# Kizuna42/office-person-detection-vit

Measured on AMD Instinct MI355X. Metric: frames/sec (Phase-2 DETR detect) at 800x1333 batch 8, higher is better.
Workload: dtype f16

## Files before the change

office_person_detection_vit_amd/csrc/kernels_btail3.hip:

```cpp
#include <hip/hip_runtime.h>
#include "opd_kernels.h"
#include "opd_elem.h"

typedef elem_t half8 __attribute__((ext_vector_type(8)));
typedef float float4v __attribute__((ext_vector_type(4)));
typedef unsigned int uint2v __attribute__((ext_vector_type(2)));
typedef unsigned int uint4v __attribute__((ext_vector_type(4)));

namespace {

constexpr int ROW_BYTES = 128;

__device__ __forceinline__ int swz(int row, int chunk) { return row * ROW_BYTES + ((chunk ^ (row & 7)) << 4); }

__device__ __forceinline__ int xcd_logical_block(int bid, int nblocks) {
    const int q = nblocks >> 3, r = nblocks & 7;
    const int x = bid & 7, k = bid >> 3;
    return (x < r ? x * (q + 1) : r * (q + 1) + (x - r) * q) + k;
}
__device__ __forceinline__ int xcd_logical_block_rev(int bid, int nblocks) {
    const int q = nblocks >> 3, r = nblocks & 7;
    const int x = bid & 7, k = bid >> 3;
    return (x < r ? x * (q + 1) + q - k : r * (q + 1) + (x - r) * q + q - 1 - k);
}
__device__ __forceinline__ int fdiv(const int m, const FastDiv& f) { return f.one ? m : (int)(__umulhi((unsigned)m, f.mul) >> f.shift); }

__device__ __forceinline__ unsigned pack2h(float a, float b) {
    typedef elem_t half2v __attribute__((ext_vector_type(2)));
    half2v h;
    h[0] = (elem_t)a;
    h[1] = (elem_t)b;
    unsigned u;
    __builtin_memcpy(&u, &h, 4);
    return u;
}
__device__ __forceinline__ void unpack2h(unsigned u, float& a, float& b) {
    typedef elem_t half2v __attribute__((ext_vector_type(2)));
    half2v h;
    __builtin_memcpy(&h, &u, 4);
    a = (float)h[0];
    b = (float)h[1];
}
__device__ __forceinline__ half8 as_half8(unsigned a, unsigned b, unsigned c, unsigned d) {
    uint4v u = {a, b, c, d};
    half8 h;
    __builtin_memcpy(&h, &u, 16);
    return h;
}
template <int N_OUTSTANDING>
__device__ __forceinline__ void wait_vmcnt() {
    static_assert(N_OUTSTANDING >= 0 && N_OUTSTANDING <= 63, "vmcnt range");
    asm volatile("s_waitcnt vmcnt(%0)" ::"n"(N_OUTSTANDING) : "memory");
}
__device__ __forceinline__ void compiler_fence() { asm volatile("" ::: "memory"); }
__device__ __forceinline__ void lds_barrier() { asm volatile("s_waitcnt lgkmcnt(0)\n\ts_barrier" ::: "memory"); }

constexpr int W2BUF = 0, W3BUF = 65536, XBUF = 131072, EXBUF = 98304;
constexpr int STAGE_BYTES = 49152;
constexpr int LDS_BYTES = 163840;

template <int C3, bool TRACE = false>
__global__ __launch_bounds__(512) void btail256_kernel(BtailParams p) {
#if defined(__HIP_DEVICE_COMPILE__)
    unsigned long long tstamp[16] = {};
    auto stamp = [&](const int i) {
        if constexpr (TRACE) asm volatile("s_memtime %0\n\ts_waitcnt lgkmcnt(0)" : "=s"(tstamp[i])::"memory");
    };
    if constexpr (TRACE) asm volatile("s_memrealtime %0\n\ts_waitcnt lgkmcnt(0)" : "=s"(tstamp[0])::"memory");
    stamp(1);
    extern __shared__ __attribute__((aligned(16))) unsigned char smem[];
    constexpr int C1 = 256, C2 = 1024, NCH = C2 / 64;
    static_assert(C3 == 0 || C3 == 256, "reduce width");
    const int tid = threadIdx.x;
    const int lane = tid & 63;
    const int wave = __builtin_amdgcn_readfirstlane(tid >> 6);
    const int pair = wave >> 1, half = wave & 1;
    const int g = lane >> 4, li = lane & 15;
    const int m_base = (p.rev ? xcd_logical_block_rev(blockIdx.x, gridDim.x) : xcd_logical_block(blockIdx.x, gridDim.x)) * 128;

    const int lrow = lane >> 3;
    const int lchunk = (lane & 7) ^ lrow;
    const unsigned backoff = (unsigned)(p.W + 1) * (unsigned)C1 * 2u;
    const __amdgpu_buffer_rsrc_t rsrc_a = __builtin_amdgcn_make_buffer_rsrc(
        const_cast<char*>(reinterpret_cast<const char*>(p.x1)) - backoff, 0, (unsigned)((size_t)p.B * p.H * p.W * C1 * 2) + backoff, 0x00020000);
    const __amdgpu_buffer_rsrc_t rsrc_w1 = __builtin_amdgcn_make_buffer_rsrc(const_cast<f16_t*>(p.w1), 0, (unsigned)(C1 * 9 * C1 * 2), 0x00020000);
    const __amdgpu_buffer_rsrc_t rsrc_w2 = __builtin_amdgcn_make_buffer_rsrc(const_cast<f16_t*>(p.w2p), 0, (unsigned)(C2 * C1 * 2), 0x00020000);
    const __amdgpu_buffer_rsrc_t rsrc_w3 = __builtin_amdgcn_make_buffer_rsrc(const_cast<f16_t*>(C3 ? p.w3p : p.w2p), 0, (unsigned)((C3 ? C3 : 1) * C2 * 2), 0x00020000);
    unsigned rowoff[2], rowmask[2], woff1[4], woff2[4], woff3[4];
    {
        const int ohw = p.OH * p.OW;
#pragma unroll
        for (int i = 0; i < 2; ++i) {
            const int m = m_base + (wave * 2 + i) * 8 + lrow;
            const bool okm = m < p.M;
            const int mm = okm ? m : 0;
            const int b = fdiv(mm, p.fd_ohw);
            const int r = mm - b * ohw;
            const int oh = fdiv(r, p.fd_ow);
            const int ow = r - oh * p.OW;
            rowoff[i] = (unsigned)(((b * p.H + oh * p.stride) * p.W + ow * p.stride) * C1) * 2u + (unsigned)lchunk * 16u;
            unsigned kwmask = 0, mask = 0;
#pragma unroll
            for (int kw = 0; kw < 3; ++kw)
                if ((unsigned)(ow * p.stride - 1 + kw) < (unsigned)p.W) kwmask |= 1u << kw;
#pragma unroll
            for (int kh = 0; kh < 3; ++kh)
                if ((unsigned)(oh * p.stride - 1 + kh) < (unsigned)p.H) mask |= kwmask << (kh * 3);
            rowmask[i] = okm ? mask : 0u;
        }
#pragma unroll
        for (int i = 0; i < 4; ++i) {
            const int q = wave * 4 + i;
            woff1[i] = (unsigned)((q * 8 + lrow) * (9 * C1)) * 2u + (unsigned)lchunk * 16u;
            woff2[i] = (unsigned)(((q & 7) * 8 + lrow) * C1 + (q >> 3) * 64) * 2u + (unsigned)lchunk * 16u;
            woff3[i] = (unsigned)((q * 8 + lrow) * C2) * 2u + (unsigned)lchunk * 16u;
        }
    }
    constexpr int kpc = C1 / 64;
    constexpr int nk = 9 * kpc;
    int tap_kh = 0, tap_kw = 0, tap_c = 0;
    int is_tap = 0, is_soff_a = 0, is_ks = 0;
    auto begin_issue = [&](int ks) {
        is_tap = tap_kh * 3 + tap_kw;
        is_soff_a = ((tap_kh * p.W + tap_kw) * C1 + tap_c * 64) * 2;
        is_ks = ks;
        if (++tap_c == kpc) {
            tap_c = 0;
            if (++tap_kw == 3) { tap_kw = 0; ++tap_kh; }
        }
    };
    auto issue_piece = [&](int i, int stage_off) {
        unsigned char* As = smem + stage_off;
        if (i < 2) {
            const unsigned vo = ((rowmask[i] >> is_tap) & 1u) ? rowoff[i] : 0x80000000u;
            __builtin_amdgcn_raw_ptr_buffer_load_lds(rsrc_a, (__attribute__((address_space(3))) void*)(As + (wave * 2 + i) * 1024), 16, vo, is_soff_a, 0, 0);
        } else {
            __builtin_amdgcn_raw_ptr_buffer_load_lds(rsrc_w1, (__attribute__((address_space(3))) void*)(As + 16384 + (wave * 4 + i - 2) * 1024), 16, woff1[i - 2], is_ks * 128, 0, 0);
        }
    };
    auto issue_main = [&](int ks, int stage_off) {
        begin_issue(ks);
#pragma unroll
        for (int i = 0; i < 6; ++i) issue_piece(i, stage_off);
    };
    auto issue_w2_piece = [&](int j, int i) {
        unsigned char* dst = smem + W2BUF + (j & 1) * 32768;
        __builtin_amdgcn_raw_ptr_buffer_load_lds(rsrc_w2, (__attribute__((address_space(3))) void*)(dst + (wave * 4 + i) * 1024), 16, woff2[i], j * (64 * C1 * 2), 0, 0);
    };
    auto issue_w3_piece = [&](int j, int i) {
        if constexpr (C3 > 0) {
            unsigned char* dst = smem + W3BUF + (j & 1) * 32768;
            __builtin_amdgcn_raw_ptr_buffer_load_lds(rsrc_w3, (__attribute__((address_space(3))) void*)(dst + (wave * 4 + i) * 1024), 16, woff3[i], j * 128, 0, 0);
        }
    };

    const int pr_m = m_base + pair * 32 + (g & 1) * 16 + li;
    const bool has_res = p.res != nullptr && !(p.dbg & 4);
    const unsigned y_bytes = (unsigned)((size_t)p.M * C2 * 2);
    const __amdgpu_buffer_rsrc_t rsrc_r = __builtin_amdgcn_make_buffer_rsrc(const_cast<f16_t*>(has_res ? p.res : p.x1), 0, has_res ? y_bytes : 0u, 0x00020000);
    const __amdgpu_buffer_rsrc_t rsrc_y = __builtin_amdgcn_make_buffer_rsrc(p.y, 0, (p.dbg & 2) ? 0u : y_bytes, 0x00020000);
    const unsigned pr_off = (unsigned)pr_m * (unsigned)(C2 * 2) + (unsigned)(half * 32 + (g >> 1) * 8) * 2u;
    auto load_res = [&](int j, uint4v (&r)[2]) {
#pragma unroll
        for (int nt = 0; nt < 2; ++nt) r[nt] = __builtin_amdgcn_raw_buffer_load_b128(rsrc_r, pr_off + (unsigned)(j * 64 + nt * 16) * 2u, 0, 0);
    };

    stamp(2);
    issue_main(0, 0);
    issue_main(1, STAGE_BYTES);
    float4v acc1[8][2];
#pragma unroll
    for (int nt = 0; nt < 8; ++nt) {
        const float4v b = *reinterpret_cast<const float4v*>(p.b1 + half * 128 + nt * 16 + g * 4);
        acc1[nt][0] = b;
        acc1[nt][1] = b;
    }
#pragma unroll
    for (int nt = 0; nt < 8; ++nt) asm volatile("" : "+v"(acc1[nt][0]), "+v"(acc1[nt][1]));
    const int group = wave >> 2;
    half8 xf[2][2], wf[2][8];
    auto read_frags = [&](int stage_off) {
        const unsigned char* As = smem + stage_off;
        const unsigned char* Ws = As + 16384;
#pragma unroll
        for (int kk = 0; kk < 2; ++kk) {
#pragma unroll
            for (int mt = 0; mt < 2; ++mt) xf[kk][mt] = *reinterpret_cast<const half8*>(As + swz(pair * 32 + mt * 16 + li, kk * 4 + g));
#pragma unroll
            for (int nt = 0; nt < 8; ++nt) wf[kk][nt] = *reinterpret_cast<const half8*>(Ws + swz(half * 128 + nt * 16 + li, kk * 4 + g));
        }
    };
    auto mfma_phase = [&](auto&& between) {
        __builtin_amdgcn_s_setprio(1);
#pragma unroll
        for (int kk = 0; kk < 2; ++kk)
#pragma unroll
            for (int nt = 0; nt < 8; ++nt) {
#pragma unroll
                for (int mt = 0; mt < 2; ++mt) acc1[nt][mt] = OPD_MFMA_16x16x32(wf[kk][nt], xf[kk][mt], acc1[nt][mt]);
                if ((nt & 3) == 3) {
                    __builtin_amdgcn_sched_barrier(0);
                    between(kk * 2 + (nt >> 2));
                    __builtin_amdgcn_sched_barrier(0);
                }
            }
        __builtin_amdgcn_s_setprio(0);
        lds_barrier();
    };
    auto no_issue = [](int) {};
    static_assert(nk % 3 == 0, "stage bookkeeping below assumes the last k-step sits in stage 2");
    wait_vmcnt<6>();
    lds_barrier();
    if (group == 1) lds_barrier();
    int st_cur = 0, st_next2 = 2 * STAGE_BYTES;
#pragma unroll 1
    for (int ks = 0; ks + 2 < nk; ++ks) {
        read_frags(st_cur);
        compiler_fence();
        begin_issue(ks + 2);
#pragma unroll
        for (int i = 0; i < 2; ++i) issue_piece(i, st_next2);
        wait_vmcnt<2>();
        lds_barrier();
        mfma_phase([&](int slot) { issue_piece(2 + slot, st_next2); });
        st_cur = st_cur == 2 * STAGE_BYTES ? 0 : st_cur + STAGE_BYTES;
        st_next2 = st_next2 == 2 * STAGE_BYTES ? 0 : st_next2 + STAGE_BYTES;
    }
    float4v acc2[2][2];
    auto load_bias2 = [&](int j) {
#pragma unroll
        for (int nt = 0; nt < 2; ++nt) acc2[nt][0] = *reinterpret_cast<const float4v*>(p.b2 + j * 64 + half * 32 + nt * 16 + g * 4);
    };
    float4v accz[C3 ? 8 : 1][2];
    read_frags(STAGE_BYTES);
    compiler_fence();
#pragma unroll
    for (int i = 0; i < 4; ++i) issue_w2_piece(0, i);
    wait_vmcnt<4>();
    lds_barrier();
    mfma_phase(no_issue);
    read_frags(2 * STAGE_BYTES);
    compiler_fence();
#pragma unroll
    for (int i = 0; i < 4; ++i) issue_w2_piece(1, i);
#pragma unroll
    for (int i = 0; i < 4; ++i) issue_w3_piece(0, i);
    compiler_fence();
    load_bias2(0);
    if constexpr (C3 > 0) {
#pragma unroll
        for (int nt = 0; nt < 8; ++nt) accz[nt][0] = *reinterpret_cast<const float4v*>(p.b3 + half * 128 + nt * 16 + g * 4);
    }
    uint4v res[3][2];
    load_res(0, res[0]);
    load_res(1, res[1]);
    compiler_fence();
    lds_barrier();
    mfma_phase(no_issue);
    if (group == 0) lds_barrier();
    wait_vmcnt<0>();
    if constexpr (C3 > 0) {
#pragma unroll
        for (int nt = 0; nt < 8; ++nt) {
            asm volatile("" : "+v"(accz[nt][0]));
            accz[nt][1] = accz[nt][0];
        }
    }
    lds_barrier();
    stamp(3);

    half8 a1[2][8];
#pragma unroll
    for (int mt = 0; mt < 2; ++mt)
#pragma unroll
        for (int kb = 0; kb < 4; ++kb) {
            float4v u = acc1[2 * kb][mt], v = acc1[2 * kb + 1][mt];
#pragma unroll
            for (int r = 0; r < 4; ++r) {
                u[r] = u[r] > 0.f ? u[r] : 0.f;
                v[r] = v[r] > 0.f ? v[r] : 0.f;
            }
            a1[mt][kb] = as_half8(pack2h(u[0], u[1]), pack2h(u[2], u[3]), pack2h(v[0], v[1]), pack2h(v[2], v[3]));
            *reinterpret_cast<half8*>(smem + EXBUF + wave * 8192 + (mt * 4 + kb) * 1024 + lane * 16) = a1[mt][kb];
        }
    lds_barrier();
#pragma unroll
    for (int mt = 0; mt < 2; ++mt)
#pragma unroll
        for (int kb = 0; kb < 4; ++kb) {
            const half8 own = a1[mt][kb];
            const half8 oth = *reinterpret_cast<const half8*>(smem + EXBUF + (wave ^ 1) * 8192 + (mt * 4 + kb) * 1024 + lane * 16);
            a1[mt][kb] = half ? oth : own;
            a1[mt][4 + kb] = half ? own : oth;
        }
    lds_barrier();
    stamp(4);
    if (p.dbg & 8) return;

#pragma unroll
    for (int j = 0; j < NCH; ++j) {
        const unsigned char* W2s = smem + W2BUF + (j & 1) * 32768;
#pragma unroll
        for (int nt = 0; nt < 2; ++nt) acc2[nt][1] = acc2[nt][0];
        {
            auto w2frag = [&](int t, int nt) {
                const int kb = t;
                return *reinterpret_cast<const half8*>(W2s + (kb >> 1) * 8192 + swz(half * 32 + nt * 16 + li, (kb & 1) * 4 + g));
            };
            half8 ring[3][2];
#pragma unroll
            for (int t = 0; t < 2; ++t)
#pragma unroll
                for (int nt = 0; nt < 2; ++nt) ring[t][nt] = w2frag(t, nt);
            __builtin_amdgcn_s_setprio(1);
#pragma unroll
            for (int t = 0; t < 8; ++t) {
                if (t + 2 < 8) {
#pragma unroll
                    for (int nt = 0; nt < 2; ++nt) ring[(t + 2) % 3][nt] = w2frag(t + 2, nt);
                }
#pragma unroll
                for (int nt = 0; nt < 2; ++nt)
#pragma unroll
                    for (int mt = 0; mt < 2; ++mt) acc2[nt][mt] = OPD_MFMA_16x16x32(ring[t % 3][nt], a1[mt][t], acc2[nt][mt]);
                __builtin_amdgcn_sched_barrier(0);
            }
            __builtin_amdgcn_s_setprio(0);
        }
        uint4v (&res_cur)[2] = res[j % 3];
        unsigned pk[2][2][2];
        uint4v yo[2];
#pragma unroll
        for (int nt = 0; nt < 2; ++nt) {
            float4v v0 = acc2[nt][0], v1 = acc2[nt][1];
            {
                uint4v r = res_cur[nt];
                asm volatile("" : "+v"(r));
                const uint2v s0 = __builtin_amdgcn_permlane16_swap(r[0], r[2], false, false);
                const uint2v s1 = __builtin_amdgcn_permlane16_swap(r[1], r[3], false, false);
                float a, b;
                unpack2h(s0[0], a, b); v0[0] += a; v0[1] += b;
                unpack2h(s1[0], a, b); v0[2] += a; v0[3] += b;
                unpack2h(s0[1], a, b); v1[0] += a; v1[1] += b;
                unpack2h(s1[1], a, b); v1[2] += a; v1[3] += b;
            }
#pragma unroll
            for (int r = 0; r < 4; ++r) {
                v0[r] = v0[r] > 0.f ? v0[r] : 0.f;
                v1[r] = v1[r] > 0.f ? v1[r] : 0.f;
            }
            pk[nt][0][0] = pack2h(v0[0], v0[1]);
            pk[nt][0][1] = pack2h(v0[2], v0[3]);
            pk[nt][1][0] = pack2h(v1[0], v1[1]);
            pk[nt][1][1] = pack2h(v1[2], v1[3]);
            const uint2v s0 = __builtin_amdgcn_permlane16_swap(pk[nt][0][0], pk[nt][1][0], false, false);
            const uint2v s1 = __builtin_amdgcn_permlane16_swap(pk[nt][0][1], pk[nt][1][1], false, false);
            yo[nt] = uint4v{s0[0], s1[0], s0[1], s1[1]};
        }
        half8 yf[2][2];
        if constexpr (C3 > 0) {
#pragma unroll
            for (int mt = 0; mt < 2; ++mt) {
                yf[0][mt] = as_half8(pk[0][mt][0], pk[0][mt][1], pk[1][mt][0], pk[1][mt][1]);
                *reinterpret_cast<half8*>(smem + XBUF + (j & 1) * 16384 + wave * 2048 + mt * 1024 + lane * 16) = yf[0][mt];
            }
        }
        wait_vmcnt<0>();
        lds_barrier();
#pragma unroll
        for (int nt = 0; nt < 2; ++nt) __builtin_amdgcn_raw_buffer_store_b128(yo[nt], rsrc_y, pr_off + (unsigned)(j * 64 + nt * 16) * 2u, 0, 0);
        if (j + 2 < NCH) load_res(j + 2, res[(j + 2) % 3]);
        if (j + 1 < NCH) load_bias2(j + 1);
        compiler_fence();
        if constexpr (C3 > 0) {
            const unsigned char* W3s = smem + W3BUF + (j & 1) * 32768;
#pragma unroll
            for (int mt = 0; mt < 2; ++mt) {
                const half8 oth = *reinterpret_cast<const half8*>(smem + XBUF + (j & 1) * 16384 + (wave ^ 1) * 2048 + mt * 1024 + lane * 16);
                const half8 own = yf[0][mt];
                yf[0][mt] = half ? oth : own;
                yf[1][mt] = half ? own : oth;
            }
            auto w3frag = [&](int idx) {
                const int kb = idx >> 3;
                return *reinterpret_cast<const half8*>(W3s + swz(half * 128 + (idx & 7) * 16 + li, kb * 4 + g));
            };
            half8 ring[4];
#pragma unroll
            for (int i = 0; i < 4; ++i) ring[i] = w3frag(i);
#pragma unroll
            for (int idx = 0; idx < 16; ++idx) {
                const half8 wf = ring[idx & 3];
#pragma unroll
                for (int mt = 0; mt < 2; ++mt) accz[idx & 7][mt] = OPD_MFMA_16x16x32(wf, yf[idx >> 3][mt], accz[idx & 7][mt]);
                if (idx + 4 < 16) ring[idx & 3] = w3frag(idx + 4);
                __builtin_amdgcn_sched_barrier(0);
                if (p.dbg & 16) {}
                else if (idx < 4) { if (j + 1 < NCH) issue_w3_piece(j + 1, idx); }
                else if (idx < 8) { if (j + 2 < NCH) issue_w2_piece(j + 2, idx - 4); }
                __builtin_amdgcn_sched_barrier(0);
            }
        } else {
            if (j + 2 < NCH) {
#pragma unroll
                for (int i = 0; i < 4; ++i) issue_w2_piece(j + 2, i);
            }
            compiler_fence();
        }
        if (j & 1) stamp(5 + (j >> 1));
    }

    if constexpr (C3 > 0) {
        const __amdgpu_buffer_rsrc_t rsrc_z = __builtin_amdgcn_make_buffer_rsrc(p.z, 0, (p.dbg & 2) ? 0u : (unsigned)((size_t)p.M * C3 * 2), 0x00020000);
        const unsigned zoff = (unsigned)pr_m * (unsigned)(C3 * 2) + (unsigned)(half * 128 + (g >> 1) * 8) * 2u;
#pragma unroll
        for (int nt = 0; nt < 8; ++nt) {
            float4v v0 = accz[nt][0], v1 = accz[nt][1];
#pragma unroll
            for (int r = 0; r < 4; ++r) {
                v0[r] = v0[r] > 0.f ? v0[r] : 0.f;
                v1[r] = v1[r] > 0.f ? v1[r] : 0.f;
            }
            const uint2v s0 = __builtin_amdgcn_permlane16_swap(pack2h(v0[0], v0[1]), pack2h(v1[0], v1[1]), false, false);
            const uint2v s1 = __builtin_amdgcn_permlane16_swap(pack2h(v0[2], v0[3]), pack2h(v1[2], v1[3]), false, false);
            const uint4v o = {s0[0], s1[0], s0[1], s1[1]};
            __builtin_amdgcn_raw_buffer_store_b128(o, rsrc_z, zoff + (unsigned)(nt * 16) * 2u, 0, 0);
        }
    }
    if constexpr (TRACE) {
        stamp(13);
        asm volatile("s_waitcnt vmcnt(0)" ::: "memory");
        stamp(14);
        asm volatile("s_memrealtime %0\n\ts_waitcnt lgkmcnt(0)" : "=s"(tstamp[15])::"memory");
        if (threadIdx.x == 0 && p.trace) {
#pragma unroll
            for (int i = 0; i < 16; ++i) p.trace[(size_t)blockIdx.x * 16 + i] = tstamp[i];
        }
    }
#endif
}

template <int C3, bool TRACE = false>
// ... 20 lines not shown
```

office_person_detection_vit_amd/csrc/kernels_btail.hip:

```cpp
#include <hip/hip_runtime.h>
#include "opd_kernels.h"
#include "opd_elem.h"

typedef elem_t half8 __attribute__((ext_vector_type(8)));
typedef float float4v __attribute__((ext_vector_type(4)));
typedef unsigned int uint2v __attribute__((ext_vector_type(2)));
typedef unsigned int uint4v __attribute__((ext_vector_type(4)));

namespace {

constexpr int ROW_BYTES = 128;
constexpr int NW = 4;

__device__ __forceinline__ int swz(int row, int chunk) { return row * ROW_BYTES + ((chunk ^ (row & 7)) << 4); }

__device__ __forceinline__ int xcd_logical_block(int bid, int nblocks) {
    const int q = nblocks >> 3, r = nblocks & 7;
    const int x = bid & 7, k = bid >> 3;
    return (x < r ? x * (q + 1) : r * (q + 1) + (x - r) * q) + k;
}

__device__ __forceinline__ int own_row(const int rho) { return (rho & ~31) | (((rho >> 2) & 3) << 3) | (((rho >> 4) & 1) << 2) | (rho & 3); }
__device__ __forceinline__ int own_ch(const int nt, const int g) { return (nt >> 1) * 32 + g * 8 + (nt & 1) * 4; }

// ... 30 lines not shown
    return h;
}

template <int N_OUTSTANDING>
__device__ __forceinline__ void wait_vmcnt() {
    static_assert(N_OUTSTANDING >= 0 && N_OUTSTANDING <= 63, "vmcnt range");
    asm volatile("s_waitcnt vmcnt(%0)" ::"n"(N_OUTSTANDING) : "memory");
}
__device__ __forceinline__ void compiler_fence() { asm volatile("" ::: "memory"); }

template <int C1, int C3, bool RDMA, bool SC = false, bool TRACE = false, int RC = 0>
__global__ __launch_bounds__(64 * NW, 8 / NW) void btail_kernel(BtailParams p) {
#if defined(__HIP_DEVICE_COMPILE__)
    unsigned long long tstamp[16] = {};
    auto stamp = [&](const int i) {
        if constexpr (TRACE) asm volatile("s_memtime %0\n\ts_waitcnt lgkmcnt(0)" : "=s"(tstamp[i])::"memory");
    };
    if constexpr (TRACE) asm volatile("s_memrealtime %0\n\ts_waitcnt lgkmcnt(0)" : "=s"(tstamp[0])::"memory");
    stamp(1);
    static_assert(!RDMA || C1 == 64, "residual staging buffers are budgeted for C1 == 64 (80 KiB of LDS per workgroup)");
    static_assert(!RDMA || RC == 0, "a rebuilt residual is not staged");
    static_assert(!SC || (C1 == 64 && !RDMA), "fused shortcut: 64-channel tails only; it replaces the residual");
    extern __shared__ __attribute__((aligned(16))) unsigned char smem[];
    constexpr int C2 = 4 * C1;
    constexpr int NT1 = C1 / 16;
    constexpr int KK1 = C1 / 32;
    constexpr int BM = 32 * NW;
    constexpr int A_BYTES = BM * ROW_BYTES;
    constexpr int RC_BYTES = RC ? 2 * 64 * ROW_BYTES : 0;
    constexpr int W1_PIECES = C1 / (8 * NW);
    constexpr int NCH = C2 / 64;
    constexpr int W2C_BYTES = 64 * C1 * 2;
    constexpr int W2_PIECES = W2C_BYTES / (1024 * NW);
    constexpr int W3_PIECES = C3 / (8 * NW);
    constexpr int SC_PIECES = 8 / NW;
    static_assert(W1_PIECES >= 1 && W2_PIECES >= 1 && (C3 == 0 || W3_PIECES >= 1), "every wave stages at least one piece of every operand");
    constexpr int NT3 = C3 / 16;
    constexpr int WSC_BYTES = SC ? 64 * ROW_BYTES : 0;
    constexpr int CHUNK_BYTES = W2C_BYTES + C3 * ROW_BYTES + WSC_BYTES + RC_BYTES;
    constexpr int STAGE_BYTES = (A_BYTES + C1 * ROW_BYTES) > CHUNK_BYTES ? (A_BYTES + C1 * ROW_BYTES) : CHUNK_BYTES;
    static_assert(RC == 0 || (RC == 1 && C1 == 64 && !RDMA && !SC), "residual rebuild: second block of stage 1");

    const int tid = threadIdx.x;
    const int lane = tid & 63;
    const int wave = __builtin_amdgcn_readfirstlane(tid >> 6);
    const int g = lane >> 4, li = lane & 15;
    const int m_base = (p.rev ? xcd_logical_block_rev(blockIdx.x, gridDim.x) : xcd_logical_block(blockIdx.x, gridDim.x)) * BM;
    const int wm0 = m_base + wave * 32;

    const int lrow = lane >> 3;
    const int lchunk = (lane & 7) ^ lrow;
    const unsigned backoff = (unsigned)(p.W + 1) * (unsigned)C1 * 2u;
    const __amdgpu_buffer_rsrc_t rsrc_a = __builtin_amdgcn_make_buffer_rsrc(
        const_cast<char*>(reinterpret_cast<const char*>(p.x1)) - backoff, 0, (unsigned)((size_t)p.B * p.H * p.W * C1 * 2) + backoff, 0x00020000);
    const __amdgpu_buffer_rsrc_t rsrc_w1 = __builtin_amdgcn_make_buffer_rsrc(const_cast<f16_t*>(p.w1), 0, (unsigned)(C1 * 9 * C1 * 2), 0x00020000);
    const __amdgpu_buffer_rsrc_t rsrc_w2 = __builtin_amdgcn_make_buffer_rsrc(const_cast<f16_t*>(p.w2p), 0, (unsigned)(C2 * C1 * 2), 0x00020000);
    const __amdgpu_buffer_rsrc_t rsrc_w3 = __builtin_amdgcn_make_buffer_rsrc(const_cast<f16_t*>(C3 ? p.w3p : p.w2p), 0, (unsigned)((C3 ? C3 : 1) * C2 * 2), 0x00020000);
    const __amdgpu_buffer_rsrc_t rsrc_sc = __builtin_amdgcn_make_buffer_rsrc(const_cast<f16_t*>(SC ? p.wsc : RC ? p.rc_wsc : p.w2p), 0, (unsigned)(C2 * 64 * 2), 0x00020000);
    const __amdgpu_buffer_rsrc_t rsrc_rw = __builtin_amdgcn_make_buffer_rsrc(const_cast<f16_t*>(RC ? p.rc_w2 : p.w2p), 0, (unsigned)(C2 * 64 * 2), 0x00020000);
    unsigned rowoff[4], rowmask[4], woff1[W1_PIECES], woff2[W2_PIECES], woff3[W3_PIECES ? W3_PIECES : 1], woffsc[2];
#pragma unroll
    for (int i = 0; i < 2; ++i)
        woffsc[i] = (unsigned)(own_row(((wave * SC_PIECES + i) & 7) * 8 + lrow) * 64) * 2u + (unsigned)lchunk * 16u;
    {
        const int ohw = p.OH * p.OW;
#pragma unroll
        for (int i = 0; i < 4; ++i) {
            const int m = m_base + (wave * 4 + i) * 8 + lrow;
            const bool okm = m < p.M;
            const int mm = okm ? m : 0;
            const int b = fdiv(mm, p.fd_ohw);
            const int r = mm - b * ohw;
// ... 46 lines not shown
        }
    };
    auto issue_chunk = [&](int j, int buf) {
        unsigned char* W2s = smem + buf * STAGE_BYTES;
#pragma unroll
        for (int i = 0; i < W2_PIECES; ++i)
            __builtin_amdgcn_raw_ptr_buffer_load_lds(rsrc_w2, (__attribute__((address_space(3))) void*)(W2s + (wave * W2_PIECES + i) * 1024),
                                                     16, woff2[i], j * (64 * C1 * 2), 0, 0);
        if constexpr (C3 > 0) {
            unsigned char* W3s = W2s + W2C_BYTES;
#pragma unroll
            for (int i = 0; i < W3_PIECES; ++i)
                __builtin_amdgcn_raw_ptr_buffer_load_lds(rsrc_w3, (__attribute__((address_space(3))) void*)(W3s + (wave * W3_PIECES + i) * 1024),
                                                         16, woff3[i], j * 128, 0, 0);
        }
        if constexpr (SC) {
            unsigned char* Wscs = W2s + W2C_BYTES + C3 * ROW_BYTES;
#pragma unroll
            for (int i = 0; i < SC_PIECES; ++i)
                __builtin_amdgcn_raw_ptr_buffer_load_lds(rsrc_sc, (__attribute__((address_space(3))) void*)(Wscs + (wave * SC_PIECES + i) * 1024), 16,
                                                         woffsc[i], j * (64 * 64 * 2), 0, 0);
        }
        if constexpr (RC) {
            unsigned char* Wr = W2s + W2C_BYTES + C3 * ROW_BYTES;
#pragma unroll
            for (int i = 0; i < SC_PIECES; ++i) {
                __builtin_amdgcn_raw_ptr_buffer_load_lds(rsrc_rw, (__attribute__((address_space(3))) void*)(Wr + (wave * SC_PIECES + i) * 1024), 16,
                                                         woffsc[i], j * (64 * 64 * 2), 0, 0);
                __builtin_amdgcn_raw_ptr_buffer_load_lds(rsrc_sc, (__attribute__((address_space(3))) void*)(Wr + 8192 + (wave * SC_PIECES + i) * 1024), 16,
                                                         woffsc[i], j * (64 * 64 * 2), 0, 0);
            }
        }
    };
    const bool pr_ok[2] = {wm0 + li < p.M, wm0 + 16 + li < p.M};
    bool y_ok[2] = {pr_ok[0] && p.y != nullptr, pr_ok[1] && p.y != nullptr};
    if (p.y_stride2) {
#pragma unroll
        for (int mt = 0; mt < 2; ++mt) {
            const int m = wm0 + mt * 16 + li;
            const int r = m - fdiv(m, p.fd_ohw) * (p.OH * p.OW);
            const int oh = fdiv(r, p.fd_ow), ow = r - oh * p.OW;
            y_ok[mt] = y_ok[mt] && !((oh | ow) & 1);
        }
    }
    const size_t pr_row[2] = {(size_t)(wm0 + li) * C2 + g * 8, (size_t)(wm0 + 16 + li) * C2 + g * 8};
    constexpr int RES_BUF = NW * 4096;
    unsigned char* const res_lds = smem + 2 * STAGE_BYTES + wave * 4096;
    const __amdgpu_buffer_rsrc_t rsrc_r = __builtin_amdgcn_make_buffer_rsrc(
        const_cast<f16_t*>(p.res ? p.res : p.x1), 0, p.res ? (unsigned)((size_t)p.M * C2 * 2) : 0u, 0x00020000);
    const unsigned res_voff = (unsigned)((wm0 + lrow) * C2) * 2u + (unsigned)lchunk * 16u;
    auto issue_res = [&](int j) {
#pragma unroll
        for (int i = 0; i < 4; ++i)
            __builtin_amdgcn_raw_ptr_buffer_load_lds(rsrc_r, (__attribute__((address_space(3))) void*)(res_lds + (j & 1) * RES_BUF + i * 1024), 16,
                                                     res_voff + (unsigned)(i * 8 * C2 * 2), j * 128, 0, 0);
    };
    const bool has_res = RC ? true : (!SC && p.res != nullptr && !(p.dbg & 4));
    const bool res_dma = RDMA && has_res;
    auto load_res = [&](int j, uint4 (&r)[4]) {
        if constexpr (RDMA) {
            if (has_res) issue_res(j);
        } else {
#pragma unroll
            for (int i = 0; i < 4; ++i) {
                r[i] = make_uint4(0u, 0u, 0u, 0u);
                if (has_res && pr_ok[i & 1]) r[i] = *reinterpret_cast<const uint4*>(p.res + pr_row[i & 1] + j * 64 + (i >> 1) * 32);
// ... 71 lines not shown
    for (int mt = 0; mt < 2; ++mt)
#pragma unroll
        for (int kk = 0; kk < KK1; ++kk) {
            float4v u = acc1[2 * kk][mt], v = acc1[2 * kk + 1][mt];
#pragma unroll
            for (int r = 0; r < 4; ++r) {
                u[r] = u[r] > 0.f ? u[r] : 0.f;
                v[r] = v[r] > 0.f ? v[r] : 0.f;
            }
            a1[mt][kk] = as_half8(pack2h(u[0], u[1]), pack2h(u[2], u[3]), pack2h(v[0], v[1]), pack2h(v[2], v[3]));
        }

    if (p.a1_out) {
#pragma unroll
        for (int mt = 0; mt < 2; ++mt)
#pragma unroll
            for (int kk = 0; kk < KK1; ++kk)
                if (pr_ok[mt]) *reinterpret_cast<half8*>(p.a1_out + (size_t)(wm0 + mt * 16 + li) * C1 + kk * 32 + g * 8) = a1[mt][kk];
    }

    float4v accz[NT3 ? NT3 : 1][2];
    if constexpr (C3 > 0) {
#pragma unroll
        for (int nt = 0; nt < NT3; ++nt) {
            const float4v b = *reinterpret_cast<const float4v*>(p.b3 + own_ch(nt, g));
            accz[nt][0] = b;
            accz[nt][1] = b;
        }
    }

    if (p.dbg & 8) return;
#pragma unroll
    for (int j = 0; j < NCH; ++j) {
        const int buf = (nk + j) & 1;
        uint4 (&res_cur)[4] = res[j % 3];
        if (j + 1 < NCH) issue_chunk(j + 1, buf ^ 1);
        compiler_fence();
        if constexpr (RDMA) {
            if (has_res) {
#pragma unroll
                for (int i = 0; i < 4; ++i)
                    res_cur[i] = *reinterpret_cast<const uint4*>(res_lds + (j & 1) * RES_BUF + swz((i & 1) * 16 + li, (i >> 1) * 4 + g));
                asm volatile("s_waitcnt lgkmcnt(0)" ::: "memory");
                if (j + 2 < NCH) issue_res(j + 2);
            }
        } else if constexpr (RC == 0) {
            if (j + 2 < NCH) load_res(j + 2, res[(j + 2) % 3]);
        }
        compiler_fence();
        const unsigned char* W2s = smem + buf * STAGE_BYTES;
        if constexpr (RC != 0) {
            const unsigned char* Wr = W2s + W2C_BYTES + C3 * ROW_BYTES;
            float4v accr[4][2];
#pragma unroll
            for (int nt = 0; nt < 4; ++nt) {
                const float4v b = *reinterpret_cast<const float4v*>(p.rc_b + j * 64 + own_ch(nt, g));
                accr[nt][0] = b;
                accr[nt][1] = b;
            }
#pragma unroll
            for (int half = 0; half < 2; ++half)
#pragma unroll
                for (int kk = 0; kk < 2; ++kk) {
                    half8 wf[4];
#pragma unroll
                    for (int nt = 0; nt < 4; ++nt) wf[nt] = *reinterpret_cast<const half8*>(Wr + half * 8192 + swz(nt * 16 + li, kk * 4 + g));
#pragma unroll
                    for (int nt = 0; nt < 4; ++nt)
#pragma unroll
// ... 39 lines not shown
                for (int nt = 0; nt < 4; ++nt) wf[nt] = *reinterpret_cast<const half8*>(Wscs + swz(nt * 16 + li, kk * 4 + g));
#pragma unroll
                for (int nt = 0; nt < 4; ++nt)
#pragma unroll
                    for (int mt = 0; mt < 2; ++mt) acc2[nt][mt] = OPD_MFMA_16x16x32(wf[nt], xs[mt][kk], acc2[nt][mt]);
            }
        }
        half8 yf[2][2];
#pragma unroll
        for (int q = 0; q < 2; ++q)
#pragma unroll
            for (int mt = 0; mt < 2; ++mt) {
                float4v v0 = acc2[2 * q][mt], v1 = acc2[2 * q + 1][mt];
                if (has_res) {
                    const uint4 r = res_cur[2 * q + mt];
                    float a, b;
                    unpack2h(r.x, a, b); v0[0] += a; v0[1] += b;
                    unpack2h(r.y, a, b); v0[2] += a; v0[3] += b;
                    unpack2h(r.z, a, b); v1[0] += a; v1[1] += b;
                    unpack2h(r.w, a, b); v1[2] += a; v1[3] += b;
                }
#pragma unroll
                for (int r = 0; r < 4; ++r) {
                    v0[r] = v0[r] > 0.f ? v0[r] : 0.f;
                    v1[r] = v1[r] > 0.f ? v1[r] : 0.f;
                }
                yf[q][mt] = as_half8(pack2h(v0[0], v0[1]), pack2h(v0[2], v0[3]), pack2h(v1[0], v1[1]), pack2h(v1[2], v1[3]));
            }
        if constexpr (C3 > 0) {
            const unsigned char* W3s = W2s + W2C_BYTES;
#pragma unroll
            for (int kk = 0; kk < 2; ++kk) {
#pragma unroll
                for (int nt = 0; nt < NT3; ++nt) {
                    const half8 wf = *reinterpret_cast<const half8*>(W3s + swz(nt * 16 + li, kk * 4 + g));
#pragma unroll
                    for (int mt = 0; mt < 2; ++mt) accz[nt][mt] = OPD_MFMA_16x16x32(wf, yf[kk][mt], accz[nt][mt]);
                }
            }
        }
        if (j + 1 < NCH) {
            if (res_dma && j + 2 < NCH) wait_vmcnt<4>();
            else wait_vmcnt<0>();
            __builtin_amdgcn_s_barrier();
        }
#pragma unroll
        for (int q = 0; q < 2; ++q)
#pragma unroll
            for (int mt = 0; mt < 2; ++mt)
                if (y_ok[mt] && !(p.dbg & 2)) *reinterpret_cast<half8*>(p.y + pr_row[mt] + j * 64 + q * 32) = yf[q][mt];
        stamp(4 + j);
    }

    if constexpr (C3 > 0) {
#pragma unroll
        for (int q = 0; q < NT3 / 2; ++q)
#pragma unroll
            for (int mt = 0; mt < 2; ++mt) {
                float4v v0 = accz[2 * q][mt], v1 = accz[2 * q + 1][mt];
#pragma unroll
                for (int r = 0; r < 4; ++r) {
                    v0[r] = v0[r] > 0.f ? v0[r] : 0.f;
                    v1[r] = v1[r] > 0.f ? v1[r] : 0.f;
                }
                if (pr_ok[mt] && !(p.dbg & 2))
                    *reinterpret_cast<uint4*>(p.z + (size_t)(wm0 + mt * 16 + li) * C3 + q * 32 + g * 8) =
                        make_uint4(pack2h(v0[0], v0[1]), pack2h(v0[2], v0[3]), pack2h(v1[0], v1[1]), pack2h(v1[2], v1[3]));
            }
    }
    if constexpr (TRACE) {
// ... 81 lines not shown
```

Measured before the change: 3093.

## Shrink btail epilogue chunks to 32 columns with triple-buffered W2/W3 and async residual loads

Restructures the conv2/conv3 epilogue loop from 16 chunks of 64 output channels into 32 stages of 32, with a three-slot ring for the W2 and W3 weight tiles. Residuals now stream into LDS through buffer_load_lds and the bias is staged once in LDS. A per-stage counted vmcnt wait replaces the full wait_vmcnt<0> drain on every iteration. The goal is deeper prefetch and less exposed global-memory latency per stage, at the cost of twice as many barriers and stages with fewer MFMAs each. It also changes the LDS layout.

```diff
diff --git a/office_person_detection_vit_amd/csrc/kernels_btail3.hip b/office_person_detection_vit_amd/csrc/kernels_btail3.hip
--- a/office_person_detection_vit_amd/csrc/kernels_btail3.hip
+++ b/office_person_detection_vit_amd/csrc/kernels_btail3.hip
@@ -52,10 +52,21 @@
     static_assert(N_OUTSTANDING >= 0 && N_OUTSTANDING <= 63, "vmcnt range");
     asm volatile("s_waitcnt vmcnt(%0)" ::"n"(N_OUTSTANDING) : "memory");
 }
+__device__ __forceinline__ void wait_vmcnt_n(const int n) {
+    switch (n) {
+        case 0: wait_vmcnt<0>(); break;
+        case 1: wait_vmcnt<1>(); break;
+        case 2: wait_vmcnt<2>(); break;
+        case 3: wait_vmcnt<3>(); break;
+        case 4: wait_vmcnt<4>(); break;
+        default: wait_vmcnt<5>(); break;
+    }
+}
 __device__ __forceinline__ void compiler_fence() { asm volatile("" ::: "memory"); }
 __device__ __forceinline__ void lds_barrier() { asm volatile("s_waitcnt lgkmcnt(0)\n\ts_barrier" ::: "memory"); }
 
-constexpr int W2BUF = 0, W3BUF = 65536, XBUF = 131072, EXBUF = 98304;
+constexpr int W2BUF = 0, W3BUF = 49152, RBUF = 98304, XBUF = 114688, BBUF = 131072, EXBUF = 98304;
+constexpr int SLOT_BYTES = 16384;
 constexpr int STAGE_BYTES = 49152;
 constexpr int LDS_BYTES = 163840;
 
@@ -69,7 +80,7 @@
     if constexpr (TRACE) asm volatile("s_memrealtime %0\n\ts_waitcnt lgkmcnt(0)" : "=s"(tstamp[0])::"memory");
     stamp(1);
     extern __shared__ __attribute__((aligned(16))) unsigned char smem[];
-    constexpr int C1 = 256, C2 = 1024, NCH = C2 / 64;
+    constexpr int C1 = 256, C2 = 1024;
     static_assert(C3 == 0 || C3 == 256, "reduce width");
     const int tid = threadIdx.x;
     const int lane = tid & 63;
@@ -86,7 +97,7 @@
     const __amdgpu_buffer_rsrc_t rsrc_w1 = __builtin_amdgcn_make_buffer_rsrc(const_cast<f16_t*>(p.w1), 0, (unsigned)(C1 * 9 * C1 * 2), 0x00020000);
     const __amdgpu_buffer_rsrc_t rsrc_w2 = __builtin_amdgcn_make_buffer_rsrc(const_cast<f16_t*>(p.w2p), 0, (unsigned)(C2 * C1 * 2), 0x00020000);
     const __amdgpu_buffer_rsrc_t rsrc_w3 = __builtin_amdgcn_make_buffer_rsrc(const_cast<f16_t*>(C3 ? p.w3p : p.w2p), 0, (unsigned)((C3 ? C3 : 1) * C2 * 2), 0x00020000);
-    unsigned rowoff[2], rowmask[2], woff1[4], woff2[4], woff3[4];
+    unsigned rowoff[2], rowmask[2], woff1[4], woff2[2], woff3[2];
     {
         const int ohw = p.OH * p.OW;
 #pragma unroll
@@ -112,8 +123,12 @@
         for (int i = 0; i < 4; ++i) {
             const int q = wave * 4 + i;
             woff1[i] = (unsigned)((q * 8 + lrow) * (9 * C1)) * 2u + (unsigned)lchunk * 16u;
-            woff2[i] = (unsigned)(((q & 7) * 8 + lrow) * C1 + (q >> 3) * 64) * 2u + (unsigned)lchunk * 16u;
-            woff3[i] = (unsigned)((q * 8 + lrow) * C2) * 2u + (unsigned)lchunk * 16u;
+        }
+#pragma unroll
+        for (int i = 0; i < 2; ++i) {
+            const int q = wave * 2 + i;
+            woff2[i] = (unsigned)(((q & 3) * 8 + lrow) * C1 + (q >> 2) * 64) * 2u + (unsigned)lchunk * 16u;
+            woff3[i] = (unsigned)((2 * (q * 8 + lrow) + (lchunk >> 2)) * C2 + (lchunk & 3) * 8) * 2u;
         }
     }
     constexpr int kpc = C1 / 64;
@@ -143,14 +158,14 @@
 #pragma unroll
         for (int i = 0; i < 6; ++i) issue_piece(i, stage_off);
     };
-    auto issue_w2_piece = [&](int j, int i) {
-        unsigned char* dst = smem + W2BUF + (j & 1) * 32768;
-        __builtin_amdgcn_raw_ptr_buffer_load_lds(rsrc_w2, (__attribute__((address_space(3))) void*)(dst + (wave * 4 + i) * 1024), 16, woff2[i], j * (64 * C1 * 2), 0, 0);
-    };
-    auto issue_w3_piece = [&](int j, int i) {
+    auto issue_w2_piece = [&](int s, int i) {
+        unsigned char* dst = smem + W2BUF + (s % 3) * SLOT_BYTES;
+        __builtin_amdgcn_raw_ptr_buffer_load_lds(rsrc_w2, (__attribute__((address_space(3))) void*)(dst + (wave * 2 + i) * 1024), 16, woff2[i], s * (32 * C1 * 2), 0, 0);
+    };
+    auto issue_w3_piece = [&](int s, int i) {
         if constexpr (C3 > 0) {
-            unsigned char* dst = smem + W3BUF + (j & 1) * 32768;
-            __builtin_amdgcn_raw_ptr_buffer_load_lds(rsrc_w3, (__attribute__((address_space(3))) void*)(dst + (wave * 4 + i) * 1024), 16, woff3[i], j * 128, 0, 0);
+            unsigned char* dst = smem + W3BUF + (s % 3) * SLOT_BYTES;
+            __builtin_amdgcn_raw_ptr_buffer_load_lds(rsrc_w3, (__attribute__((address_space(3))) void*)(dst + (wave * 2 + i) * 1024), 16, woff3[i], s * 64, 0, 0);
         }
     };
 
@@ -159,10 +174,11 @@
     const unsigned y_bytes = (unsigned)((size_t)p.M * C2 * 2);
     const __amdgpu_buffer_rsrc_t rsrc_r = __builtin_amdgcn_make_buffer_rsrc(const_cast<f16_t*>(has_res ? p.res : p.x1), 0, has_res ? y_bytes : 0u, 0x00020000);
     const __amdgpu_buffer_rsrc_t rsrc_y = __builtin_amdgcn_make_buffer_rsrc(p.y, 0, (p.dbg & 2) ? 0u : y_bytes, 0x00020000);
-    const unsigned pr_off = (unsigned)pr_m * (unsigned)(C2 * 2) + (unsigned)(half * 32 + (g >> 1) * 8) * 2u;
-    auto load_res = [&](int j, uint4v (&r)[2]) {
-#pragma unroll
-        for (int nt = 0; nt < 2; ++nt) r[nt] = __builtin_amdgcn_raw_buffer_load_b128(rsrc_r, pr_off + (unsigned)(j * 64 + nt * 16) * 2u, 0, 0);
+    const unsigned pr_off = (unsigned)pr_m * (unsigned)(C2 * 2) + (unsigned)(half * 16 + (g >> 1) * 8) * 2u;
+    auto load_res = [&](int s) { return __builtin_amdgcn_raw_buffer_load_b128(rsrc_r, pr_off + (unsigned)(s * 64), 0, 0); };
+    auto issue_res = [&](int s) {
+        __builtin_amdgcn_raw_ptr_buffer_load_lds(rsrc_r, (__attribute__((address_space(3))) void*)(smem + RBUF + (s & 1) * 8192 + wave * 1024), 16,
+                                                 pr_off + (unsigned)(s * 64), 0, 0, 0);
     };
 
     stamp(2);
@@ -226,39 +242,37 @@
         st_cur = st_cur == 2 * STAGE_BYTES ? 0 : st_cur + STAGE_BYTES;
         st_next2 = st_next2 == 2 * STAGE_BYTES ? 0 : st_next2 + STAGE_BYTES;
     }
-    float4v acc2[2][2];
-    auto load_bias2 = [&](int j) {
-#pragma unroll
-        for (int nt = 0; nt < 2; ++nt) acc2[nt][0] = *reinterpret_cast<const float4v*>(p.b2 + j * 64 + half * 32 + nt * 16 + g * 4);
-    };
+    float4v acc2n;
     float4v accz[C3 ? 8 : 1][2];
     read_frags(STAGE_BYTES);
     compiler_fence();
 #pragma unroll
-    for (int i = 0; i < 4; ++i) issue_w2_piece(0, i);
+    for (int i = 0; i < 2; ++i) issue_w2_piece(0, i);
+#pragma unroll
+    for (int i = 0; i < 2; ++i) issue_w2_piece(1, i);
     wait_vmcnt<4>();
     lds_barrier();
-    mfma_phase(no_issue);
+    mfma_phase([&](int slot) { if (slot < 2) issue_w2_piece(2, slot); });
     read_frags(2 * STAGE_BYTES);
     compiler_fence();
 #pragma unroll
-    for (int i = 0; i < 4; ++i) issue_w2_piece(1, i);
-#pragma unroll
-    for (int i = 0; i < 4; ++i) issue_w3_piece(0, i);
+    for (int i = 0; i < 2; ++i) issue_w3_piece(0, i);
+#pragma unroll
+    for (int i = 0; i < 2; ++i) issue_w3_piece(1, i);
     compiler_fence();
-    load_bias2(0);
+    acc2n = *reinterpret_cast<const float4v*>(p.b2 + half * 16 + g * 4);
+    float2 b2v = reinterpret_cast<const float2*>(p.b2)[tid];
     if constexpr (C3 > 0) {
 #pragma unroll
         for (int nt = 0; nt < 8; ++nt) accz[nt][0] = *reinterpret_cast<const float4v*>(p.b3 + half * 128 + nt * 16 + g * 4);
     }
-    uint4v res[3][2];
-    load_res(0, res[0]);
-    load_res(1, res[1]);
+    uint4v res0 = load_res(0), res1 = load_res(1);
     compiler_fence();
     lds_barrier();
     mfma_phase(no_issue);
     if (group == 0) lds_barrier();
     wait_vmcnt<0>();
+    asm volatile("" : "+v"(res0), "+v"(res1), "+v"(acc2n), "+v"(b2v));
     if constexpr (C3 > 0) {
 #pragma unroll
         for (int nt = 0; nt < 8; ++nt) {
@@ -294,120 +308,105 @@
             a1[mt][4 + kb] = half ? own : oth;
         }
     lds_barrier();
+    reinterpret_cast<float2*>(smem + BBUF)[tid] = b2v;
     stamp(4);
     if (p.dbg & 8) return;
 
-#pragma unroll
-    for (int j = 0; j < NCH; ++j) {
-        const unsigned char* W2s = smem + W2BUF + (j & 1) * 32768;
-#pragma unroll
-        for (int nt = 0; nt < 2; ++nt) acc2[nt][1] = acc2[nt][0];
+    constexpr int NST = C2 / 32;
+    auto n_req = [](int s) {
+        return (s + 2 < NST ? 1 + (C3 > 0 ? 2 : 0) : 0) + (s + 3 < NST ? 2 : 0);
+    };
+#pragma unroll
+    for (int s = 0; s < NST; ++s) {
+        const unsigned char* W2s = smem + W2BUF + (s % 3) * SLOT_BYTES;
+        float4v acc2[2] = {acc2n, acc2n};
         {
-            auto w2frag = [&](int t, int nt) {
-                const int kb = t;
-                return *reinterpret_cast<const half8*>(W2s + (kb >> 1) * 8192 + swz(half * 32 + nt * 16 + li, (kb & 1) * 4 + g));
-            };
-            half8 ring[3][2];
-#pragma unroll
-            for (int t = 0; t < 2; ++t)
-#pragma unroll
-                for (int nt = 0; nt < 2; ++nt) ring[t][nt] = w2frag(t, nt);
+            auto w2frag = [&](int kb) { return *reinterpret_cast<const half8*>(W2s + (kb >> 1) * 4096 + swz(half * 16 + li, (kb & 1) * 4 + g)); };
+            half8 ring[3];
+            ring[0] = w2frag(0);
+            ring[1] = w2frag(1);
             __builtin_amdgcn_s_setprio(1);
 #pragma unroll
             for (int t = 0; t < 8; ++t) {
-                if (t + 2 < 8) {
-#pragma unroll
-                    for (int nt = 0; nt < 2; ++nt) ring[(t + 2) % 3][nt] = w2frag(t + 2, nt);
-                }
-#pragma unroll
-                for (int nt = 0; nt < 2; ++nt)
-#pragma unroll
-                    for (int mt = 0; mt < 2; ++mt) acc2[nt][mt] = OPD_MFMA_16x16x32(ring[t % 3][nt], a1[mt][t], acc2[nt][mt]);
+                if (t + 2 < 8) ring[(t + 2) % 3] = w2frag(t + 2);
+#pragma unroll
+                for (int mt = 0; mt < 2; ++mt) acc2[mt] = OPD_MFMA_16x16x32(ring[t % 3], a1[mt][t], acc2[mt]);
                 __builtin_amdgcn_sched_barrier(0);
             }
             __builtin_amdgcn_s_setprio(0);
         }
-        uint4v (&res_cur)[2] = res[j % 3];
-        unsigned pk[2][2][2];
-        uint4v yo[2];
-#pragma unroll
-        for (int nt = 0; nt < 2; ++nt) {
-            float4v v0 = acc2[nt][0], v1 = acc2[nt][1];
-            {
-                uint4v r = res_cur[nt];
-                asm volatile("" : "+v"(r));
-                const uint2v s0 = __builtin_amdgcn_permlane16_swap(r[0], r[2], false, false);
-                const uint2v s1 = __builtin_amdgcn_permlane16_swap(r[1], r[3], false, false);
-                float a, b;
-                unpack2h(s0[0], a, b); v0[0] += a; v0[1] += b;
-                unpack2h(s1[0], a, b); v0[2] += a; v0[3] += b;
-                unpack2h(s0[1], a, b); v1[0] += a; v1[1] += b;
-                unpack2h(s1[1], a, b); v1[2] += a; v1[3] += b;
-            }
-#pragma unroll
-            for (int r = 0; r < 4; ++r) {
-                v0[r] = v0[r] > 0.f ? v0[r] : 0.f;
-                v1[r] = v1[r] > 0.f ? v1[r] : 0.f;
-            }
-            pk[nt][0][0] = pack2h(v0[0], v0[1]);
-            pk[nt][0][1] = pack2h(v0[2], v0[3]);
-            pk[nt][1][0] = pack2h(v1[0], v1[1]);
-            pk[nt][1][1] = pack2h(v1[2], v1[3]);
-            const uint2v s0 = __builtin_amdgcn_permlane16_swap(pk[nt][0][0], pk[nt][1][0], false, false);
-            const uint2v s1 = __builtin_amdgcn_permlane16_swap(pk[nt][0][1], pk[nt][1][1], false, false);
-            yo[nt] = uint4v{s0[0], s1[0], s0[1], s1[1]};
-        }
-        half8 yf[2][2];
+        if (s > 0) wait_vmcnt_n(n_req(s - 1));
+        uint4v r = s == 0 ? res0 : s == 1 ? res1 : *reinterpret_cast<const uint4v*>(smem + RBUF + (s & 1) * 8192 + wave * 1024 + lane * 16);
+        asm volatile("" : "+v"(r));
+        unsigned pk[2][2];
+        uint4v yo;
+        {
+            float4v v0 = acc2[0], v1 = acc2[1];
+            const uint2v s0 = __builtin_amdgcn_permlane16_swap(r[0], r[2], false, false);
+            const uint2v s1 = __builtin_amdgcn_permlane16_swap(r[1], r[3], false, false);
+            float a, b;
+            unpack2h(s0[0], a, b); v0[0] += a; v0[1] += b;
+            unpack2h(s1[0], a, b); v0[2] += a; v0[3] += b;
+            unpack2h(s0[1], a, b); v1[0] += a; v1[1] += b;
+            unpack2h(s1[1], a, b); v1[2] += a; v1[3] += b;
+#pragma unroll
+            for (int q = 0; q < 4; ++q) {
+                v0[q] = v0[q] > 0.f ? v0[q] : 0.f;
+                v1[q] = v1[q] > 0.f ? v1[q] : 0.f;
+            }
+            pk[0][0] = pack2h(v0[0], v0[1]);
+            pk[0][1] = pack2h(v0[2], v0[3]);
+            pk[1][0] = pack2h(v1[0], v1[1]);
+            pk[1][1] = pack2h(v1[2], v1[3]);
+            const uint2v t0 = __builtin_amdgcn_permlane16_swap(pk[0][0], pk[1][0], false, false);
+            const uint2v t1 = __builtin_amdgcn_permlane16_swap(pk[0][1], pk[1][1], false, false);
+            yo = uint4v{t0[0], t1[0], t0[1], t1[1]};
+        }
+        unsigned char* xch = smem + XBUF + (s & 1) * 8192;
         if constexpr (C3 > 0) {
 #pragma unroll
+            for (int mt = 0; mt < 2; ++mt) *reinterpret_cast<uint2v*>(xch + wave * 1024 + mt * 512 + lane * 8) = uint2v{pk[mt][0], pk[mt][1]};
+        }
+        lds_barrier();
+        __builtin_amdgcn_raw_buffer_store_b128(yo, rsrc_y, pr_off + (unsigned)(s * 64), 0, 0);
+        compiler_fence();
+        if (s + 1 < NST) acc2n = *reinterpret_cast<const float4v*>(smem + BBUF + ((s + 1) * 32 + half * 16 + g * 4) * 4);
+        auto issue = [&](int k) {
+            if (k == 0) { if (s + 2 < NST) issue_res(s + 2); }
+            else if (k < 3) { if (s + 2 < NST && !(p.dbg & 16)) issue_w3_piece(s + 2, k - 1); }
+            else if (s + 3 < NST && !(p.dbg & 16)) issue_w2_piece(s + 3, k - 3);
+        };
+        if constexpr (C3 > 0) {
+            half8 yb[2];
+#pragma unroll
             for (int mt = 0; mt < 2; ++mt) {
-                yf[0][mt] = as_half8(pk[0][mt][0], pk[0][mt][1], pk[1][mt][0], pk[1][mt][1]);
-                *reinterpret_cast<half8*>(smem + XBUF + (j & 1) * 16384 + wave * 2048 + mt * 1024 + lane * 16) = yf[0][mt];
-            }
-        }
-        wait_vmcnt<0>();
-        lds_barrier();
-#pragma unroll
-        for (int nt = 0; nt < 2; ++nt) __builtin_amdgcn_raw_buffer_store_b128(yo[nt], rsrc_y, pr_off + (unsigned)(j * 64 + nt * 16) * 2u, 0, 0);
-        if (j + 2 < NCH) load_res(j + 2, res[(j + 2) % 3]);
-        if (j + 1 < NCH) load_bias2(j + 1);
-        compiler_fence();
-        if constexpr (C3 > 0) {
-            const unsigned char* W3s = smem + W3BUF + (j & 1) * 32768;
-#pragma unroll
-            for (int mt = 0; mt < 2; ++mt) {
-                const half8 oth = *reinterpret_cast<const half8*>(smem + XBUF + (j & 1) * 16384 + (wave ^ 1) * 2048 + mt * 1024 + lane * 16);
-                const half8 own = yf[0][mt];
-                yf[0][mt] = half ? oth : own;
-                yf[1][mt] = half ? own : oth;
-            }
+                const uint2v oth = *reinterpret_cast<const uint2v*>(xch + (wave ^ 1) * 1024 + mt * 512 + lane * 8);
+                yb[mt] = half ? as_half8(oth[0], oth[1], pk[mt][0], pk[mt][1]) : as_half8(pk[mt][0], pk[mt][1], oth[0], oth[1]);
+            }
+            const unsigned char* W3s = smem + W3BUF + (s % 3) * SLOT_BYTES;
             auto w3frag = [&](int idx) {
-                const int kb = idx >> 3;
-                return *reinterpret_cast<const half8*>(W3s + swz(half * 128 + (idx & 7) * 16 + li, kb * 4 + g));
+                const int n = half * 128 + idx * 16 + li;
+                return *reinterpret_cast<const half8*>(W3s + swz(n >> 1, (n & 1) * 4 + g));
             };
             half8 ring[4];
 #pragma unroll
             for (int i = 0; i < 4; ++i) ring[i] = w3frag(i);
 #pragma unroll
-            for (int idx = 0; idx < 16; ++idx) {
+            for (int idx = 0; idx < 8; ++idx) {
                 const half8 wf = ring[idx & 3];
 #pragma unroll
-                for (int mt = 0; mt < 2; ++mt) accz[idx & 7][mt] = OPD_MFMA_16x16x32(wf, yf[idx >> 3][mt], accz[idx & 7][mt]);
-                if (idx + 4 < 16) ring[idx & 3] = w3frag(idx + 4);
+                for (int mt = 0; mt < 2; ++mt) accz[idx][mt] = OPD_MFMA_16x16x32(wf, yb[mt], accz[idx][mt]);
+                if (idx + 4 < 8) ring[idx & 3] = w3frag(idx + 4);
                 __builtin_amdgcn_sched_barrier(0);
-                if (p.dbg & 16) {}
-                else if (idx < 4) { if (j + 1 < NCH) issue_w3_piece(j + 1, idx); }
-                else if (idx < 8) { if (j + 2 < NCH) issue_w2_piece(j + 2, idx - 4); }
+                if (idx < 5) issue(idx);
                 __builtin_amdgcn_sched_barrier(0);
             }
         } else {
-            if (j + 2 < NCH) {
-#pragma unroll
-                for (int i = 0; i < 4; ++i) issue_w2_piece(j + 2, i);
-            }
+#pragma unroll
+            for (int k = 0; k < 5; ++k) issue(k);
             compiler_fence();
         }
-        if (j & 1) stamp(5 + (j >> 1));
+        if ((s & 3) == 3) stamp(5 + (s >> 2));
     }
 
     if constexpr (C3 > 0) {
```

After: 3111, median of 6. About the same (+0.6%).

## Split W3 staging into half steps to shrink bottleneck-tail LDS stage buffers

Applied to the files above, without the earlier changes.

When the per-chunk operand set (W2 chunk plus full W3 slab) exceeds the stage-1 buffer size, the W3 projection is split into two halves. The lower half travels with the W2 chunk and the upper half is streamed into the other stage buffer during compute. This shrinks STAGE_BYTES and so LDS use per workgroup, which can allow more resident workgroups. In exchange it adds an extra vmcnt(0) wait and barrier per chunk and serializes the next-chunk prefetch behind the upper-half MFMAs.

```diff
diff --git a/office_person_detection_vit_amd/csrc/kernels_btail.hip b/office_person_detection_vit_amd/csrc/kernels_btail.hip
--- a/office_person_detection_vit_amd/csrc/kernels_btail.hip
+++ b/office_person_detection_vit_amd/csrc/kernels_btail.hip
@@ -86,12 +86,16 @@
     constexpr int NCH = C2 / 64;
     constexpr int W2C_BYTES = 64 * C1 * 2;
     constexpr int W2_PIECES = W2C_BYTES / (1024 * NW);
-    constexpr int W3_PIECES = C3 / (8 * NW);
+    constexpr bool SPLIT3 = 64 * C1 * 2 + C3 * ROW_BYTES > (32 * NW + C1) * ROW_BYTES;
+    static_assert(!SPLIT3 || (!RDMA && !SC && RC == 0 && !TRACE), "half steps: plain residual tails only (every wait is a vmcnt(0))");
+    constexpr int C3H = SPLIT3 ? C3 / 2 : C3;
+    constexpr int W3_PIECES = C3H / (8 * NW);
     constexpr int SC_PIECES = 8 / NW;
     static_assert(W1_PIECES >= 1 && W2_PIECES >= 1 && (C3 == 0 || W3_PIECES >= 1), "every wave stages at least one piece of every operand");
     constexpr int NT3 = C3 / 16;
     constexpr int WSC_BYTES = SC ? 64 * ROW_BYTES : 0;
-    constexpr int CHUNK_BYTES = W2C_BYTES + C3 * ROW_BYTES + WSC_BYTES + RC_BYTES;
+    constexpr int CHUNK_BYTES = W2C_BYTES + C3H * ROW_BYTES + WSC_BYTES + RC_BYTES;
+    static_assert(!SPLIT3 || C3H * ROW_BYTES <= CHUNK_BYTES, "the W3-only half step fits a stage buffer");
     constexpr int STAGE_BYTES = (A_BYTES + C1 * ROW_BYTES) > CHUNK_BYTES ? (A_BYTES + C1 * ROW_BYTES) : CHUNK_BYTES;
     static_assert(RC == 0 || (RC == 1 && C1 == 64 && !RDMA && !SC), "residual rebuild: second block of stage 1");
 
@@ -204,6 +208,13 @@
             }
         }
     };
+    auto issue_w3_upper = [&](int j, int buf) {
+        unsigned char* W3s = smem + buf * STAGE_BYTES;
+#pragma unroll
+        for (int i = 0; i < W3_PIECES; ++i)
+            __builtin_amdgcn_raw_ptr_buffer_load_lds(rsrc_w3, (__attribute__((address_space(3))) void*)(W3s + (wave * W3_PIECES + i) * 1024), 16,
+                                                     woff3[i], C3H * C2 * 2 + j * 128, 0, 0);
+    };
     const bool pr_ok[2] = {wm0 + li < p.M, wm0 + 16 + li < p.M};
     bool y_ok[2] = {pr_ok[0] && p.y != nullptr, pr_ok[1] && p.y != nullptr};
     if (p.y_stride2) {
@@ -341,9 +352,10 @@
     if (p.dbg & 8) return;
 #pragma unroll
     for (int j = 0; j < NCH; ++j) {
-        const int buf = (nk + j) & 1;
+        const int buf = SPLIT3 ? (nk & 1) : ((nk + j) & 1);
         uint4 (&res_cur)[4] = res[j % 3];
-        if (j + 1 < NCH) issue_chunk(j + 1, buf ^ 1);
+        if constexpr (SPLIT3) issue_w3_upper(j, buf ^ 1);
+        else if (j + 1 < NCH) issue_chunk(j + 1, buf ^ 1);
         compiler_fence();
         if constexpr (RDMA) {
             if (has_res) {
@@ -449,10 +461,26 @@
 #pragma unroll
             for (int kk = 0; kk < 2; ++kk) {
 #pragma unroll
-                for (int nt = 0; nt < NT3; ++nt) {
+                for (int nt = 0; nt < C3H / 16; ++nt) {
                     const half8 wf = *reinterpret_cast<const half8*>(W3s + swz(nt * 16 + li, kk * 4 + g));
 #pragma unroll
                     for (int mt = 0; mt < 2; ++mt) accz[nt][mt] = OPD_MFMA_16x16x32(wf, yf[kk][mt], accz[nt][mt]);
+                }
+            }
+        }
+        if constexpr (SPLIT3) {
+            wait_vmcnt<0>();
+            __builtin_amdgcn_s_barrier();
+            if (j + 1 < NCH) issue_chunk(j + 1, buf);
+            compiler_fence();
+            const unsigned char* W3u = smem + (buf ^ 1) * STAGE_BYTES;
+#pragma unroll
+            for (int kk = 0; kk < 2; ++kk) {
+#pragma unroll
+                for (int nt = 0; nt < C3H / 16; ++nt) {
+                    const half8 wf = *reinterpret_cast<const half8*>(W3u + swz(nt * 16 + li, kk * 4 + g));
+#pragma unroll
+                    for (int mt = 0; mt < 2; ++mt) accz[C3H / 16 + nt][mt] = OPD_MFMA_16x16x32(wf, yf[kk][mt], accz[C3H / 16 + nt][mt]);
                 }
             }
         }
```

Result: slower. 3101 before, 3064 after (-1.2%).
